# focegueda1998/CALM-ViT-DTE

Measured on AMD Instinct MI355X. Metric: training images/sec (224^2, bs=256/GPU), higher is better.
Workload: dtype f32; 1 GPU; CALM-ViT small224 cls, 224x224x3 synthetic, bs=256/GPU, fp32 matmuls, fwd+loss+bwd+clip+AdamW; batch resident in HBM when the timed region starts (the trainer's H2D copy of the batch is excluded); global_batch=256, parallelism=dp1, world=1, backend=none (single process), hipgraph=False

## Files before the change

calm-vit-dte_amd/Vi_Tools_CNN_less_V2.py:

```python
from functools import partial
from typing import Callable

import torch

from . import ops
from .backend import ACT_GELU, ACT_NONE, lean_forward
from .spectral_norm import SNConv2d, SNLinear, sn_scope


class ResidualStateManager():

    def __init__(self, smooth_factor: float = 2.0, momentum: float = 0.9, mode: str = "ema"):
        super().__init__()
        self.zq_sum = None
        self.zkv_sum = None
        self.tot_kl_loss = 0.0
        self.count = 0
        self.smooth_factor = smooth_factor
        self.mode = mode
        self.momentum = momentum

    @staticmethod
    def _kl(mean, std):
        return -0.5 * torch.mean(1 + 2 * torch.log(std) - mean.pow(2) - std.pow(2))
# ... 159 lines not shown
        self.rope_q = RoPE(seq_len_new, d_rope, learned=True)
        self.rope_k = RoPE(seq_len_new, d_rope, learned=True)
        self.linear_mask = torch.nn.Sequential(
            SNLinear(seq_len_new, seq_len_new * 2, bias=True),
            GELU(),
            SNLinear(seq_len_new * 2, seq_len_new, bias=True),
        )
        self.out_proj = SNLinear(dim2, dim2)
        self.out_proj.layer_scaled = True
        self.dropout = torch.nn.Dropout(dropout)
        self.ln_2 = LayerNorm(dim2)
        self.mlp = None
        if use_mlp:
            self.mlp = torch.nn.Sequential(
                SNLinear(dim2, mlp_dim),
                GELU(),
                torch.nn.Dropout(dropout, inplace=False),
                SNLinear(mlp_dim, dim2),
            )
            self.mlp[3].layer_scaled = True

    @staticmethod
    def _seq(lin, x):
        return ops.SeqLinearFn.apply(x, lin.weight_orig, lin.weight_u, lin.weight_v, lin.sigma())

    def forward(self, input_q, input_kv=None, state_manager=None, mask=False):
        if not mask:
            raise AttributeError("'NoneType' object has no attribute 'unsqueeze' (mask=False is not a usable "
                                 "path of the reference; every caller passes mask=True)")
        with sn_scope(self):
            return self._forward(input_q, input_kv, state_manager)

    def _project_qkv(self, qz, kz, vz, out16=False):
        pq, pk, pv = self.q_proj, self.k_proj, self.v_proj
        pack = lambda *ps: [t for p_ in ps for t in (p_.weight_orig, p_.weight_u, p_.weight_v, p_.sigma())]
        same_shape = pq.weight_orig.shape == pk.weight_orig.shape == pv.weight_orig.shape
        if any(p_.bias is not None for p_ in (pq, pk, pv)) or not same_shape or not ops.GROUP_PROJECTIONS:
            return pq(qz, out16=out16), pk(kz, out16=out16), pv(vz, out16=out16)
        if qz is kz and kz is vz:
            return ops.SNLinearGroupFn.apply(qz, out16, *pack(pq, pk, pv))
        if kz is vz:
            k, v = ops.SNLinearGroupFn.apply(kz, out16, *pack(pk, pv))
            return pq(qz, out16=out16), k, v
        return pq(qz, out16=out16), pk(kz, out16=out16), pv(vz, out16=out16)

    def _forward(self, input_q, input_kv, state_manager):
        H = self.heads
        xq, residual = self.ln_q.with_skip(input_q)
        xkv = xq if input_kv is None else self.ln_kv(input_kv, gemm_only=True)
        qz = qr = xq
        kz = vz = kr = xkv
        if self.reduce:
            if self.t_reduce:
                xq = self._seq(self.t_encoder_q, xq)
                xkv = self._seq(self.t_encoder_kv, xkv)
            mv_q = self.encoder_q(xq)
            mv_kv = self.encoder_kv(xkv)
            mvh = mv_q.shape[-1] // 2
            nq = ops.draw_noise(mv_q[..., :mvh]) if self.training else None
            nkv = ops.draw_noise(mv_kv[..., :mvh]) if self.training else None
            zq, std_q, kl_q = ops.LatentFn.apply(mv_q, nq)
            zkv, std_kv, kl_kv = ops.LatentFn.apply(mv_kv, nkv)
            if state_manager is not None:
                zq, zkv = state_manager.get_sums(zq, zkv, mv_q[..., :mvh], std_q, mv_kv[..., :mvh], std_kv,
                                                 kl_q=kl_q, kl_kv=kl_kv)
            qr = qz = zq
            kz = vz = zkv
            if self.t_reduce:
                qz = self._seq(self.t_qz_upsample, qz)
                kz = self._seq(self.t_kz_upsample, kz)
                vz = self._seq(self.t_vz_upsample, vz)
                qr = self._seq(self.t_qr_proj, qr)
                kr = self._seq(self.t_kr_proj, kr)
        a16 = qz.shape[1] == kz.shape[1] and ops.use_attention16(qz.shape[1], H, self.head_dim)
        qz, kz, v = self._project_qkv(qz, kz, vz, out16=a16)
        if self.reduce:
            qr = self.qr_proj(qr, out16=a16)
            kr = self.kr_proj(kr, out16=a16)
            q = ops.RopeFn.apply(qz, qr, self.rope_q.inv_freq, H, a16)
            k = ops.RopeFn.apply(kz, kr, self.rope_k.inv_freq, H, a16)
        else:
            q = ops.RopeFn.apply(None, qz, self.rope_q.inv_freq, H, a16)
            k = ops.RopeFn.apply(None, kz, self.rope_k.inv_freq, H, a16)
        m0, m2 = self.linear_mask[0], self.linear_mask[2]
        attention = ops.LatentMaskAttention16Fn if a16 else ops.LatentMaskAttentionFn
        if not a16 and ops.use_attention_lse(q.shape[1], k.shape[1], H, self.head_dim):
            attention = ops.LatentMaskAttentionLseFn
        if lean_forward():
            x = ops.latent_mask_attention_infer(q, k, v, m0.weight_orig, m0.bias, m2.weight_orig, m2.bias,
                                                m0.sigma(), m2.sigma(), H)
        else:
            x = attention.apply(
                q, k, v, m0.weight_orig, m0.bias, m2.weight_orig, m2.bias,
                m0.weight_u, m0.weight_v, m0.sigma(), m2.weight_u, m2.weight_v, m2.sigma(), H)
        if residual.shape != (x.shape[0], x.shape[1], self.out_proj.out_features):
            if self.input_t_proj is not None:
                residual = self._seq(self.input_t_proj, residual)
            if self.input_proj is not None:
                residual = self.input_proj(residual)
        p_att = self.dropout.p if self.training else 0.0
        if p_att > 0:
            x = self.out_proj(x, ls=self.ls_att)
            x = ops.DropoutAddFn.apply(x, residual, p_att, ops.draw_dropout_key(x.device))
        else:
            x = self.out_proj(x, ls=self.ls_att, residual=residual)
        if self.mlp is None:
            return self.ln_2(x)
        y, x = self.ln_2.with_skip(x)
        l0, l3 = self.mlp[0], self.mlp[3]
        mlp_args = (y, l0.weight_orig, None, l3.weight_orig, None, self.ls_mlp, x,
                    l0.weight_u, l0.weight_v, l0.sigma(), l3.weight_u, l3.weight_v, l3.sigma())
        p_mlp = self.mlp[2].p if self.training else 0.0
        if p_mlp > 0:
            return ops.MlpFn.apply(*mlp_args, p_mlp, ops.draw_dropout_key(y.device))
        return ops.MlpFn.apply(*mlp_args, 0.0, None, lean_forward())


class CnnResidual(torch.nn.Sequential):

    def __init__(self, hidden_channels=32):
        super().__init__(
            SNConv2d(3, hidden_channels, kernel_size=1, groups=1, bias=True),
            GELU(),
            SNConv2d(hidden_channels, hidden_channels, kernel_size=3, padding=1, bias=True, groups=hidden_channels),
            GELU(),
# ... 131 lines not shown
```

calm-vit-dte_amd/_lib.py:

```python
import ctypes as C
import os

HERE = os.path.dirname(os.path.abspath(__file__))
LIB_PATH = os.environ.get("CALM_VIT_LIB") or os.path.join(HERE, "libcalmvit_hip.so")

ACT_NONE, ACT_GELU, ACT_GELU_BWD = 0, 1, 2
F32 = 0
ST_F32, ST_BF16, ST_FP8_E4M3, ST_FP8_E5M2 = 0, 1, 2, 3
E_INVAL, E_LAYOUT, E_UNSUPP = -1, -2, -3
ABI_VERSION = 7

_p = C.c_void_p
_i32 = C.c_int32
_i64 = C.c_int64
_f32 = C.c_float


class GemmArgs(C.Structure):
    _fields_ = [
        ("A", _p), ("B", _p), ("C", _p),
        ("M", _i32), ("N", _i32), ("K", _i32),
        ("batch0", _i32), ("batch1", _i32),
        ("a_rs", _i64), ("a_cs", _i64), ("a_b0", _i64), ("a_b1", _i64),
        ("b_rs", _i64), ("b_cs", _i64), ("b_b0", _i64), ("b_b1", _i64),
# ... 140 lines not shown
    "calm_attention_bwd_lse": (_i32, [_p] * 7 + [_i64] + [_p] * 4 + [_i32] * 5 + [_p]),
    "calm_attention_infer": (_i32, [_p] * 11 + [_i32] * 5 + [_p]),
    "calm_attention16_supported": (_i32, [_i32, _i32, _i32]),
    "calm_attention16_fwd": (_i32, [_p] * 16 + [_i32] * 4 + [_p]),
    "calm_attention16_bwd": (_i32, [_p] * 13 + [_i32] * 4 + [_p]),
    "calm_attention16_infer": (_i32, [_p] * 11 + [_i32] * 4 + [_p]),
    "calm_latent_fwd": (_i32, [_p, _p, _p, _p, _p, _i64, _i32, _p, _p]),
    "calm_latent_bwd": (_i32, [_p, _p, _p, _p, _p, _p, _i64, _i32, _p]),
    "calm_sn_plan": (_i32, [C.POINTER(SnLayer), _i32, _p, C.POINTER(SnPlanInfo)]),
    "calm_sn_power_iter": (_i32, [_p, C.POINTER(SnPlanInfo), _i32, _f32, _p, _p]),
    "calm_sn_weight_bwd": (_i32, [_p, _p, _p, _p, _p, _p, _p, _p, _i32, _i32, _p, _p]),
    "calm_optim_chunk_elems": (_i32, []),
    "calm_optim_step": (_i32, [_p, _i32, _p, _i32, _p, C.POINTER(OptimHparams), _p, _p, _p, _p, _p]),
    "calm_grad_accum": (_i32, [_p, _i32, _p, _i32, _p, _p, _i32, _p]),
    "calm_ema_chunk_elems": (_i32, []),
    "calm_ema_update": (_i32, [_p, _i32, _p, _i32, _f32, _i32, _p, _p, _p, _p]),
    "calm_ema_swap": (_i32, [_p, _i32, _p, _i32, _p]),
    "calm_snapshot_chunk_bytes": (_i32, []),
    "calm_snapshot_pack": (_i32, [_p, _i32, _p, _i32, _p, _i64, _p]),
    "calm_snapshot_unpack": (_i32, [_p, _i32, _p, _i32, _p, _i64, _p]),
    "calm_collate_mix": (_i32, [_p, _p, _p, _i32, _i32, _i32, _i32, _f32, _p, _p, _p, _p]),
    "calm_collate_crop_mix": (_i32, [_p, _i32, _i32, _p, _p, _p, _i32, _i32, _i32, _i32, _i32, _f32, _p, _p, _p, _p]),
    "calm_augment_collate": (_i32, [_p, _i32, _i32, _p, _p, _p, _i32, _i32, _i32, _i32, _i32, _f32, _p, _p, _p, _p]),
    "calm_resize_coeffs": (_i32, [_i32, _i32, _p, _p, _i32]),
    "calm_resize_u8": (_i32, [_p, _i64, _p, _p, _i32, _i32, _i32, _p]),
    "calm_resized_crop": (_i32, [_p, _i64, _p, _p, _i32, _i32, _i32, _i32, _p, _p, _p]),
    "calm_resized_crop_check": (_i32, [C.POINTER(RCropSample), _i64, _i32, _i32]),
    "calm_image_to_rows": (_i32, [_p, _p, _i32, _i32, _p]),
    "calm_rows_to_image": (_i32, [_p, _p, _i32, _i32, _p]),
    "calm_grid_transpose": (_i32, [_p, _p, _i32, _i32, _p]),
    "calm_dwconv3x3_fwd": (_i32, [_p, _p, _p, _p, _p, _p, _i32, _i32, _i32, _i32, _p]),
    "calm_dwconv3x3_bwd": (_i32, [_p, _p, _p, _p, _p, _p, _p, _i32, _i32, _i32, _p]),
    "calm_cnn_residual_fwd": (_i32, [_p] * 11 + [_i32, _i32, _i32, _i32, _p]),
    "calm_cnn_residual_bwd": (_i32, [_p] * 18 + [_i32, _i32, _i32, _i32, _p, _p]),
    "calm_add": (_i32, [_p, _p, _p, _i64, _p]),
    "calm_gelu_fwd": (_i32, [_p, _p, _i64, _p]),
    "calm_gelu_bwd": (_i32, [_p, _p, _p, _i64, _p]),
    "calm_colsum": (_i32, [_p, _p, _i64, _i32, _i32, _p, _p]),
    "calm_row_scale": (_i32, [_p, _p, _p, _i32, _i32, _i32, _p]),
    "calm_mean_seq_fwd": (_i32, [_p, _p, _i32, _i32, _i32, _p]),
    "calm_mean_seq_bwd": (_i32, [_p, _p, _i32, _i32, _i32, _p]),
    "calm_soft_ce_fwd": (_i32, [_p, _i64, _p, _i64, _p, _p, _p, _i32, _i32, _p, _p]),
    "calm_soft_ce_bwd": (_i32, [_p, _i64, _p, _i64, _p, _p, _p, _i32, _i32, _p]),
    "calm_huber_tokens_fwd": (_i32, [_p, _p, _f32, _p, _i32, _i32, _p, _p]),
    "calm_huber_tokens_bwd": (_i32, [_p, _p, _f32, _p, _p, _i32, _i32, _p]),
    "calm_top1_count": (_i32, [_p, _i64, _p, _p, _i32, _i32, _p]),
    "calm_eval_metrics": (_i32, [_p, _i64, _i32, _p, C.POINTER(_i32), _i32, _p, _p, _p, _i32, _i32, _p, _p]),
    "calm_recon_huber_rows_fwd": (_i32, [_p, _p, _f32, _p, _i64, _p, _p]),
    "calm_recon_huber_rows_bwd": (_i32, [_p, _p, _f32, _p, _p, _i64, _p]),
    "calm_recon_metrics": (_i32, [_p, _i32, _p, _i32, C.POINTER(_f32), C.POINTER(_f32), _f32, _i32, _p, _i32, _i32, _p, _p]),
    "calm_distill_fwd": (_i32, [_p, _i64, _p, _i64, _i32, _p, _i64, _f32, _f32, _i32, _p, _p, _p, _p, _i32, _i32, _p, _p]),
    "calm_distill_bwd": (_i32, [_p, _i64, _p, _i64, _i32, _p, _i64, _f32, _f32, _i32, _p, _p, _p, _i32, _i32, _p]),
    "calm_dropout": (_i32, [_p, _p, _p, _i64, _i64, _f32, _p, _i32, _i32, _i32, _p]),
}

_lib = None


def load():
    global _lib
    if _lib is not None:
        return _lib
    if not os.path.exists(LIB_PATH):
        raise RuntimeError(
            f"{LIB_PATH} is missing: build it with `python -c 'import __graft_entry__ as g; g.build()'` "
            "(hipcc --offload-arch=gfx950).  The CALM-ViT path has no non-HIP fallback.")
    lib = C.CDLL(LIB_PATH)
    for name, (res, args) in SIGNATURES.items():
        fn = getattr(lib, name)
        fn.restype = res
        fn.argtypes = args
    if lib.calm_abi_version() != ABI_VERSION:
        raise RuntimeError("libcalmvit_hip.so ABI version mismatch")
    _lib = lib
    return lib


def check(rc, what):
    if rc != 0:
        kind = "invalid argument/unsupported shape" if rc < 0 else "hipError_t"
        raise RuntimeError(f"{what} failed: code {rc} ({kind})")
```

calm-vit-dte_amd/backend.py:

```python
import contextlib
import ctypes as C
import os

import numpy as np
import torch

from . import _lib
from ._lib import ACT_GELU, ACT_GELU_BWD, ACT_NONE

SN_EPS = 1e-12

GEMM_WORKSPACE = os.environ.get("CALM_GEMM_WORKSPACE", "1") != "0"
BF16_STORAGE = os.environ.get("CALM_BF16_STORAGE", "1") != "0"
PRECISIONS = {"fp32": 0, "bf16": 1, "bf16x3": 2, "fp8": 1}
FP8_DTYPES = (torch.float8_e4m3fn, torch.float8_e5m2)
_precision = "fp32"


def set_matmul_precision(name):
    global _precision
    if name not in PRECISIONS:
        raise ValueError(f"unknown matmul precision {name!r}; choose from {sorted(PRECISIONS)}")
    _precision = name

# ... 38 lines not shown
def lean_forward():
    return _lean_inference and not torch.is_grad_enabled()


_loss_kernels = os.environ.get("CALM_LOSS_KERNELS", "0") not in ("", "0")


def set_loss_kernels(on):
    global _loss_kernels
    _loss_kernels = bool(on)


def get_loss_kernels():
    return _loss_kernels


def loss_kernels_take(t):
    return _loss_kernels and t.dtype == torch.float32 and (t.is_cuda or not isinstance(get_backend(), HipBackend))


def eval_kernels_take(t):
    return (_loss_kernels and t.dtype in (torch.float32, torch.bfloat16)
            and (t.is_cuda or not isinstance(get_backend(), HipBackend)))


def recon_kernels_take(tokens, target):
    return eval_kernels_take(tokens) and target.dtype == torch.float32 and target.device == tokens.device


def effective_precision():
    if torch.is_autocast_enabled("cuda"):
        dt = torch.get_autocast_dtype("cuda")
        if dt != torch.bfloat16:
            raise NotImplementedError(f"autocast dtype {dt} is not supported on this path (the reference uses bfloat16)")
        return "bf16"
    return "bf16" if _precision == "fp8" else _precision


def fp8_linears():
    return _precision == "fp8" and BF16_STORAGE


def _ptr(t, allow_none=False, bf16_ok=False, fp8_ok=False):
    if t is None:
        if allow_none:
            return None
        raise ValueError("required tensor is None")
    if not t.is_cuda:
        raise RuntimeError("CALM-ViT ops run only on the MI355X HIP path: got a CPU tensor "
                           "(there is no CPU fallback; move the model and inputs to 'cuda')")
    if t.dtype != torch.float32 and not (bf16_ok and t.dtype == torch.bfloat16) and not (fp8_ok and t.dtype in FP8_DTYPES):
        raise TypeError(f"fp32 tensor expected, got {t.dtype}")
    return t.data_ptr()


def _ptr16(t):
    if t is None or not t.is_cuda or t.dtype != torch.bfloat16 or not t.is_contiguous():
        raise TypeError("contiguous bf16 CUDA tensor expected")
    return t.data_ptr()


_ST_OF = {torch.bfloat16: _lib.ST_BF16, torch.float8_e4m3fn: _lib.ST_FP8_E4M3, torch.float8_e5m2: _lib.ST_FP8_E5M2}


def _st(t):
    if t is None:
        return _lib.ST_F32
    return _ST_OF.get(t.dtype, _lib.ST_F32)


def bf16_pipeline():
    return BF16_STORAGE and effective_precision() == "bf16"


def act_dtype(last_dim):
    return torch.bfloat16 if bf16_pipeline() and last_dim % 8 == 0 else torch.float32


_raw_stream = getattr(torch._C, "_cuda_getCurrentRawStream", None)
_cur_device = getattr(torch._C, "_cuda_getDevice", None)


def _stream():
    if _raw_stream is not None:
        return _raw_stream(_cur_device())
    return torch.cuda.current_stream().cuda_stream


def chunk_table(lengths, chunk):
    chunk0, chunk_entry = [], []
    for i, n in enumerate(lengths):
        chunk0.append(len(chunk_entry))
        chunk_entry += [i] * ((n + chunk - 1) // chunk)
    return chunk0, chunk_entry


def _disjoint(spans):
    spans = sorted(spans)
    return not any(b[0] < a[1] for a, b in zip(spans, spans[1:]))


class ChunkPlan:

    def _tables(self, rec, lengths, chunk, dev):
        chunk0, chunk_entry = chunk_table(lengths, chunk)
        rec["chunk0"] = chunk0
# ... 845 lines not shown
        if partials is None:
            part = self._partials(_lib.RED_RECON, B, S, tokens.device)
        else:
            if partials.numel() < self.recon_scratch_floats(B, S):
                raise ValueError("recon_metrics: partials is smaller than calm_reduce_scratch_floats(CALM_RED_RECON, B, S)")
            part = _ptr(partials)
        m3, s3 = (_lib.C.c_float * 3)(*[float(v) for v in mean]), (_lib.C.c_float * 3)(*[float(v) for v in std])
        _lib.check(self.lib.calm_recon_metrics(_ptr(tokens, bf16_ok=True), _st(tokens), _ptr(target), int(layout), m3, s3,
                                               float(delta), int(bool(want_ssim)), sums.data_ptr(), B, S, part, _stream()),
                   "calm_recon_metrics")

    def recon_scratch_floats(self, B, S):
        need = self._scratch_need.get((_lib.RED_RECON, B, S))
        if need is None:
            need = self._scratch_need[(_lib.RED_RECON, B, S)] = int(self.lib.calm_reduce_scratch_floats(_lib.RED_RECON, B, S))
        return need

    def dropout(self, x, residual, y, n, p, key, e0=0):
        if key is None or not key.is_cuda or key.dtype != torch.int64 or key.numel() != 2 or not key.is_contiguous():
            raise TypeError("dropout expects its key as a contiguous int64 CUDA tensor of two elements (seed, offset)")
        _lib.check(self.lib.calm_dropout(_ptr(x, bf16_ok=True), _ptr(residual, True, bf16_ok=True), _ptr(y, bf16_ok=True),
                                         n, e0, float(p), key.data_ptr(), _st(x), _st(residual), _st(y), _stream()),
                   "calm_dropout")

    def add(self, a, b, out, n):
        _lib.check(self.lib.calm_add(_ptr(a), _ptr(b), _ptr(out), n, _stream()), "calm_add")

    def gelu_fwd(self, x, y, n):
        _lib.check(self.lib.calm_gelu_fwd(_ptr(x), _ptr(y), n, _stream()), "calm_gelu_fwd")

    def gelu_bwd(self, dy, z, dz, n):
        _lib.check(self.lib.calm_gelu_bwd(_ptr(dy), _ptr(z), _ptr(dz), n, _stream()), "calm_gelu_bwd")

    def colsum(self, x, out, rows, cols):
        _lib.check(self.lib.calm_colsum(_ptr(x, bf16_ok=True), _ptr(out), rows, cols, _st(x),
                                        self._partials(_lib.RED_COLSUM, rows, cols, x.device), _stream()), "calm_colsum")

    def colsum_part(self, x, rows, cols):
        part, shape = self._own_partials(_lib.RED_COLSUM, rows, cols, x.device), _lib.ReduceShape()
        _lib.check(self.lib.calm_part_colsum(_ptr(x, bf16_ok=True), rows, cols, _st(x), _ptr(part), C.byref(shape),
                                             _stream()), "calm_part_colsum")
        return part, shape

    def row_scale(self, x, s, out, rows, cols):
        _lib.check(self.lib.calm_row_scale(_ptr(x), _ptr(s), _ptr(out, bf16_ok=True), rows, cols, _st(out), _stream()),
                   "calm_row_scale")

    def mean_seq_fwd(self, x, y, B, S, D):
        _lib.check(self.lib.calm_mean_seq_fwd(_ptr(x), _ptr(y), B, S, D, _stream()), "calm_mean_seq_fwd")

    def mean_seq_bwd(self, dy, dx, B, S, D):
        _lib.check(self.lib.calm_mean_seq_bwd(_ptr(dy), _ptr(dx), B, S, D, _stream()), "calm_mean_seq_bwd")


_backend = None


def get_backend():
    global _backend
    if _backend is None:
        _backend = HipBackend()
    return _backend


@contextlib.contextmanager
def use_backend(b):
    global _backend
    old = _backend
    _backend = b
    try:
        yield b
    finally:
        _backend = old
```

calm-vit-dte_amd/build.py:

```python
import os
import shutil
import subprocess

HERE = os.path.dirname(os.path.abspath(__file__))
CSRC = os.path.join(HERE, "csrc")
LIB = os.path.join(HERE, "libcalmvit_hip.so")
SOURCES = ["gemm.hip", "gemm_f32.hip", "gemm_bf16.hip", "gemm_bf16p_kk.hip", "gemm_bf16p_km.hip", "gemm_bf16p_mm.hip", "gemm_f32p_kk.hip", "gemm_f32p_km.hip", "gemm_f32p_mm.hip", "gemm_fp8.hip", "norm_act.hip", "spectral.hip", "tokens_conv.hip", "cnn_fused.hip",
           "attention_fused.hip", "attention_bf16.hip", "optim.hip", "accum.hip", "ema.hip", "snapshot.hip", "loss.hip", "recon.hip", "dropout.hip", "augment.hip", "resize.hip", "resized_crop.hip"]
FLAGS = ["--offload-arch=gfx950", "-O3", "-fPIC", "-std=c++17", "-Wall", "-Wno-unused-function"]


def _hipcc():
    for cand in (os.environ.get("HIPCC"), shutil.which("hipcc"), "/opt/rocm/bin/hipcc"):
        if cand and os.path.exists(cand):
            return cand
    raise RuntimeError("hipcc not found: the CALM-ViT HIP library cannot be built")


def _stale(target, deps):
    if not os.path.exists(target):
        return True
    t = os.path.getmtime(target)
    return any(os.path.getmtime(d) > t for d in deps)


def build_library(force=False, verbose=False):
    hipcc = _hipcc()
    headers = [os.path.join(CSRC, h) for h in os.listdir(CSRC) if h.endswith(".h")]
    headers.append(os.path.join(HERE, "..", "include", "calm_vit.h"))
    objdir = os.path.join(HERE, "build")
    os.makedirs(objdir, exist_ok=True)
    objs, jobs = [], []
    for src in SOURCES:
        s = os.path.join(CSRC, src)
        o = os.path.join(objdir, src.replace(".hip", ".o"))
        if force or _stale(o, [s] + headers):
            cmd = [hipcc] + FLAGS + ["-c", s, "-o", o]
            if verbose:
                print(" ".join(cmd))
            jobs.append((src, subprocess.Popen(cmd)))
        objs.append(o)
    failed = [src for src, pr in jobs if pr.wait() != 0]
    if failed:
        raise RuntimeError(f"hipcc failed for {failed}")
    if force or _stale(LIB, objs):
        cmd = [hipcc, "--offload-arch=gfx950", "-shared", "-fPIC", "-o", LIB] + objs
        if verbose:
            print(" ".join(cmd))
        subprocess.run(cmd, check=True)
    return LIB


if __name__ == "__main__":
    print(build_library(verbose=True))
```

calm-vit-dte_amd/ops.py:

```python
import math
import os
import threading

import torch
from torch.autograd import Function
from torch.autograd.function import once_differentiable

from . import _lib
from .backend import (ACT_GELU, ACT_GELU_BWD, ACT_NONE, act_dtype, bf16_pipeline, effective_precision, fp8_linears,
                      get_attention_storage, get_backend)
from .spectral_norm import W16_ATTR, W16_GEN_ATTR

_amp_fwd = torch.amp.custom_fwd(device_type="cuda")
_amp_bwd = torch.amp.custom_bwd(device_type="cuda")

GROUP_PROJECTIONS = os.environ.get("CALM_GROUP_PROJECTIONS", "1") != "0"
FUSE_LN_SKIP = os.environ.get("CALM_FUSE_LN_SKIP", "1") != "0"

_noise_override = None


def set_noise_override(fn):
    global _noise_override
    _noise_override = fn
# ... 520 lines not shown
        ctx.wops = (wop1, wop2)
        ctx.wgen = _wgen(w1, w2)
        ctx.has_b1, ctx.has_b2, ctx.has_res = b1 is not None, b2 is not None, residual is not None
        ctx.biases = (_leaf(b1), _leaf(b2))
        ctx.defer = (_deferred(w1), _deferred(w2))
        ctx.xshape = x.shape
        ctx.save_for_backward(x2, hp, hg, w1, w2, ls, u1, v1, s1, u2, v2, s2, key if ctx.p > 0 else None)
        return out

    @staticmethod
    @once_differentiable
    @_amp_bwd
    def backward(ctx, dout):
        be = get_backend()
        x2, hp, hg, w1, w2, ls, u1, v1, s1, u2, v2, s2, key = ctx.saved_tensors
        _check_wgen(ctx.wgen, w1, w2)
        N, Hd = w2.shape
        K = w1.shape[1]
        do2 = _c(dout).reshape(-1, N)
        do2g = _gop(be, do2)
        G2 = _zeros_big(w2.shape, w2)
        _lin_wgrad(be, do2g, hg, G2)
        dW2, d_ls = _sn_wbwd(be, G2, w2, u2, v2, s2, ls, defer=ctx.defer[1])
        db2 = _colsum(be, do2, ctx.biases[1]) if ctx.has_b2 else None
        wop1, wop2 = ctx.wops
        if ls is not None:
            w2l = torch.empty_like(w2 if ctx.fp8 else wop2)
            be.row_scale(w2, ls, w2l, N, Hd)
        else:
            w2l = w2 if ctx.fp8 else wop2
        dhp = torch.empty_like(hp)
        if ctx.fp8:
            _lin_dgrad8(be, do2, w2l, s2, dhp, act=ACT_GELU_BWD, aux=hp)
        else:
            _lin_dgrad(be, do2g, w2l, s2, dhp, act=ACT_GELU_BWD, aux=hp)
        if ctx.p > 0:
            be.dropout(dhp, None, dhp, dhp.numel(), ctx.p, key)
        G1 = _zeros_big(w1.shape, w1)
        _lin_wgrad(be, dhp, x2, G1)
        dW1, _ = _sn_wbwd(be, G1, w1, u1, v1, s1, defer=ctx.defer[0])
        db1 = _colsum(be, dhp, ctx.biases[0]) if ctx.has_b1 else None
        dx = None
        if ctx.needs_input_grad[0]:
            dx = torch.empty_like(x2)
            if ctx.fp8:
                _lin_dgrad8(be, dhp, w1, s1, dx)
            else:
                _lin_dgrad(be, dhp, wop1, s1, dx)
            dx = dx.view(ctx.xshape)
        dres = dout if ctx.has_res else None
        return dx, dW1, db1, dW2, db2, d_ls, dres, None, None, None, None, None, None, None, None, None


class SeqLinearFn(Function):

    @staticmethod
    @_amp_fwd
    def forward(ctx, x, w, u, v, sigma):
        be = get_backend()
        x = _c(x)
        B, S, D = x.shape
        S2 = w.shape[0]
        wop = _wop(w)
        out = torch.empty(B, S2, D, dtype=torch.float32, device=x.device)
        be.gemm(wop, x, out, S2, D, S, (S, 1, 0, 0), (1, D, S * D, 0), (D, S2 * D, 0), batch=(B, 1), inv_scale=sigma)
        ctx.defer = _deferred(w)
        ctx.wop = wop
        ctx.wgen = _wgen(w)
        ctx.save_for_backward(x, w, u, v, sigma)
        return out

    @staticmethod
    @once_differentiable
    @_amp_bwd
    def backward(ctx, dy):
        be = get_backend()
        x, w, u, v, sigma = ctx.saved_tensors
        _check_wgen(ctx.wgen, w)
        B, S, D = x.shape
        S2 = w.shape[0]
        dy = _c(dy)
        dx = None
        if ctx.needs_input_grad[0]:
            dx = torch.empty_like(x)
            be.gemm(ctx.wop, dy, dx, S, D, S2, (1, S, 0, 0), (1, D, S2 * D, 0), (D, S * D, 0), batch=(B, 1),
                    inv_scale=sigma)
        G = _zeros_big(w.shape, w)
        be.gemm(dy, x, G, S2, S, D, (D, 1, S2 * D, 0), (D, 1, S * D, 0), (S, 0, 0), batch=(B, 1), reduce_batch=True,
                accumulate=True)
        dW, _ = _sn_wbwd(be, G, w, u, v, sigma, defer=ctx.defer)
        return dx, dW, None, None, None


class RopeFn(Function):

    @staticmethod
    @_amp_fwd
    def forward(ctx, content, xr, inv_freq, H, out16=False):
        be = get_backend()
        xr = _c(xr)
        B, S, W = xr.shape
        dr = W // H
        dc = 0
        if content is not None:
            content = _c(content)
            dc = content.shape[-1] // H
        table = torch.empty(2 * S * (dr // 2), dtype=torch.float32, device=xr.device)
        out = torch.empty(B, S, H * (dc + dr), dtype=torch.bfloat16 if out16 else torch.float32, device=xr.device)
        be.rope_fwd(content, xr, inv_freq, table, out, B, S, H, dc, dr)
        ctx.dims = (B, S, H, dc, dr)
        ctx.content_dtype = content.dtype if content is not None else None
        ctx.inv_freq = _leaf(inv_freq)
        ctx.save_for_backward(xr, table)
        return out

    @staticmethod
    @once_differentiable
    @_amp_bwd
    def backward(ctx, dout):
        be = get_backend()
        xr, table = ctx.saved_tensors
        B, S, H, dc, dr = ctx.dims
        dout = _c(dout)
        d_xr = torch.empty_like(xr)
        d_content = torch.empty(B, S, H * dc, dtype=ctx.content_dtype, device=xr.device) if dc > 0 else None
        d_if = _zeros((dr // 2,), table)
        if ctx.inv_freq is not None and _tail.takes(be, ctx.inv_freq):
            part, shape = be.rope_bwd_part(dout, xr, table, d_content, d_xr, B, S, H, dc, dr)
            _tail.add_reduce(part, shape, [d_if], (ctx.inv_freq,))
        else:
            be.rope_bwd(dout, xr, table, d_content, d_xr, d_if, B, S, H, dc, dr)
        return d_content, d_xr, d_if, None, None


def _attn_mask_bwd(be, defer, dM, q, k, dq, dk, R, hp, hg, w1, w2, u1, v1, s1, u2, v2, s2, w1o=None, w2o=None,
                   fold=False, biases=(None, None)):
    w1o, w2o = w1 if w1o is None else w1o, w2 if w2o is None else w2o
    B, Sq, D = q.shape
    Skv = k.shape[1]
    dev, dt = q.device, q.dtype
    G2 = _zeros_big(w2.shape, w2)
    _lin_wgrad(be, dM, hg, G2)
    dW2, _ = _sn_wbwd(be, G2, w2, u2, v2, s2, defer=defer[1])
    db2 = _colsum(be, dM, biases[1])
# ... 621 lines not shown
```

include/calm_vit.h:

```cpp
#ifndef CALM_VIT_H
#define CALM_VIT_H

#include <stddef.h>
#include <stdint.h>

#ifdef __cplusplus
extern "C" {
#endif

#define CALM_ABI_VERSION 7

#define CALM_E_INVAL   (-1)
#define CALM_E_LAYOUT  (-2)
#define CALM_E_UNSUPP  (-3)

enum { CALM_F32 = 0, CALM_BF16 = 1, CALM_BF16X3 = 2 };
enum { CALM_ST_F32 = 0, CALM_ST_BF16 = 1, CALM_ST_FP8_E4M3 = 2, CALM_ST_FP8_E5M2 = 3 };
enum { CALM_ACT_NONE = 0, CALM_ACT_GELU = 1, CALM_ACT_GELU_BWD = 2 };

int         calm_abi_version(void);
const char* calm_build_info(void);

typedef struct calm_gemm_args {
    const void* A; const void* B; void* C;
// ... 311 lines not shown
                          void* stream);

int calm_add(const float* a, const float* b, float* out, int64_t n, void* stream);
int calm_gelu_fwd(const float* x, float* y, int64_t n, void* stream);
int calm_gelu_bwd(const float* dy, const float* z, float* dz, int64_t n, void* stream);
int calm_colsum(const void* x, float* out, int64_t rows, int32_t cols, int32_t x_type ,
                float* partials , void* stream);
int calm_row_scale(const float* x, const float* s, void* out, int32_t rows, int32_t cols, int32_t out_type ,
                   void* stream);
int calm_mean_seq_fwd(const float* x, float* y, int32_t B, int32_t S, int32_t D, void* stream);
int calm_mean_seq_bwd(const float* dy, float* dx, int32_t B, int32_t S, int32_t D, void* stream);

int calm_dropout(const void* x, const void* residual , void* y, int64_t n, int64_t e0, float p,
                 const uint64_t* key , int32_t x_type, int32_t r_type, int32_t y_type,
                 void* stream);

int calm_soft_ce_fwd(const float* logits, int64_t ld, const float* targets, int64_t td,
                     float* row_stats ,
                     float* loss , float* metrics ,
                     int32_t B, int32_t C, float* partials, void* stream);
int calm_soft_ce_bwd(const float* logits, int64_t ld, const float* targets, int64_t td, const float* row_stats,
                     const float* dloss, float* dlogits , int32_t B, int32_t C, void* stream);
int calm_huber_tokens_fwd(const float* tokens, const float* x, float delta, float* loss, int32_t B, int32_t S,
                          float* partials, void* stream);
int calm_huber_tokens_bwd(const float* tokens, const float* x, float delta, const float* dloss, float* dtokens,
                          int32_t B, int32_t S, void* stream);
int calm_top1_count(const float* logits, int64_t ld, const int64_t* labels, float* metrics, int32_t B, int32_t C, void* stream);

int calm_eval_metrics(const void* logits, int64_t ld, int32_t logits_type, const int64_t* labels, const int32_t* ks,
                      int32_t nk, int64_t* counts, double* loss_sum, int64_t* confusion , int32_t B, int32_t C,
                      float* partials, void* stream);

enum { CALM_RECON_ROWS = 0, CALM_RECON_NCHW = 1 };
int calm_recon_huber_rows_fwd(const float* tokens, const float* target, float delta, float* loss ,
                              int64_t n, float* partials, void* stream);
int calm_recon_huber_rows_bwd(const float* tokens, const float* target, float delta, const float* dloss, float* dtokens,
                              int64_t n, void* stream);
int calm_recon_metrics(const void* tokens, int32_t tokens_type, const float* target, int32_t target_layout,
                       const float* mean , const float* std , float delta, int32_t want_ssim,
                       double* sums , int32_t B, int32_t S, float* partials, void* stream);

enum { CALM_DISTILL_SOFT = 0, CALM_DISTILL_HARD = 1 };
#define CALM_DISTILL_ROW_STATS 8
int calm_distill_fwd(const float* logits, int64_t ld, const void* teacher, int64_t tld, int32_t teacher_type,
                     const float* targets, int64_t td, float temperature, float alpha, int32_t mode,
                     float* row_stats , float* loss ,
                     float* metrics , float* dmetrics , int32_t B, int32_t C,
                     float* partials, void* stream);
int calm_distill_bwd(const float* logits, int64_t ld, const void* teacher, int64_t tld, int32_t teacher_type,
                     const float* targets, int64_t td, float temperature, float alpha, int32_t mode,
                     const float* row_stats, const float* dloss , float* dlogits ,
                     int32_t B, int32_t C, void* stream);

#ifdef __cplusplus
}
#endif
#endif
```

Measured before the change: 1977 images/sec.

## Add grouped sequence-mixing linear kernels and batch shared-input token projections

Adds a dedicated HIP kernel family for sequence-axis linear layers: forward and dgrad keep the small weight in LDS and use MFMA, and wgrad splits the batch reduction across workgroups with a partials buffer. Only the wgrad route is enabled by default for short sequences. The attention block now groups sequence projections that share an input (encoder q/kv, qz/qr upsample, kz/vz upsample) into one autograd function, so the grouped path runs several weights per launch. This aims to cut launch count and the poor utilisation of generic batched GEMMs on tiny S×S weights, at the cost of extra scratch memory and a separate reduction pass.

```diff
diff --git a/calm-vit-dte_amd/Vi_Tools_CNN_less_V2.py b/calm-vit-dte_amd/Vi_Tools_CNN_less_V2.py
--- a/calm-vit-dte_amd/Vi_Tools_CNN_less_V2.py
+++ b/calm-vit-dte_amd/Vi_Tools_CNN_less_V2.py
@@ -235,8 +235,11 @@
         kz = vz = kr = xkv
         if self.reduce:
             if self.t_reduce:
-                xq = self._seq(self.t_encoder_q, xq)
-                xkv = self._seq(self.t_encoder_kv, xkv)
+                if input_kv is None:
+                    xq, xkv = ops.seq_linear_group(xq, [self.t_encoder_q, self.t_encoder_kv])
+                else:
+                    xq = self._seq(self.t_encoder_q, xq)
+                    xkv = self._seq(self.t_encoder_kv, xkv)
             mv_q = self.encoder_q(xq)
             mv_kv = self.encoder_kv(xkv)
             mvh = mv_q.shape[-1] // 2
@@ -250,10 +253,8 @@
             qr = qz = zq
             kz = vz = zkv
             if self.t_reduce:
-                qz = self._seq(self.t_qz_upsample, qz)
-                kz = self._seq(self.t_kz_upsample, kz)
-                vz = self._seq(self.t_vz_upsample, vz)
-                qr = self._seq(self.t_qr_proj, qr)
+                qz, qr = ops.seq_linear_group(zq, [self.t_qz_upsample, self.t_qr_proj])
+                kz, vz = ops.seq_linear_group(zkv, [self.t_kz_upsample, self.t_vz_upsample])
                 kr = self._seq(self.t_kr_proj, kr)
         a16 = qz.shape[1] == kz.shape[1] and ops.use_attention16(qz.shape[1], H, self.head_dim)
         qz, kz, v = self._project_qkv(qz, kz, vz, out16=a16)
diff --git a/calm-vit-dte_amd/_lib.py b/calm-vit-dte_amd/_lib.py
--- a/calm-vit-dte_amd/_lib.py
+++ b/calm-vit-dte_amd/_lib.py
@@ -216,6 +216,11 @@
     "calm_distill_fwd": (_i32, [_p, _i64, _p, _i64, _i32, _p, _i64, _f32, _f32, _i32, _p, _p, _p, _p, _i32, _i32, _p, _p]),
     "calm_distill_bwd": (_i32, [_p, _i64, _p, _i64, _i32, _p, _i64, _f32, _f32, _i32, _p, _p, _p, _i32, _i32, _p]),
     "calm_dropout": (_i32, [_p, _p, _p, _i64, _i64, _f32, _p, _i32, _i32, _i32, _p]),
+    "calm_seq_linear_supported": (_i32, [_i32, _i32, _i32, _i32]),
+    "calm_seq_linear_scratch_floats": (_i64, [_i32, _i32, _i32, _i32, _i32]),
+    "calm_seq_linear_fwd": (_i32, [_p, _p, _p, _p, _i32, _i32, _i32, _i32, _i32, _p]),
+    "calm_seq_linear_dgrad": (_i32, [_p, _p, _p, _p, _i32, _i32, _i32, _i32, _i32, _p]),
+    "calm_seq_linear_wgrad": (_i32, [_p, _p, _p, _i32, _i32, _i32, _i32, _i32, _i32, _p, _i64, _p]),
 }
 
 _lib = None
diff --git a/calm-vit-dte_amd/backend.py b/calm-vit-dte_amd/backend.py
--- a/calm-vit-dte_amd/backend.py
+++ b/calm-vit-dte_amd/backend.py
@@ -114,6 +114,12 @@
     if t.dtype != torch.float32 and not (bf16_ok and t.dtype == torch.bfloat16) and not (fp8_ok and t.dtype in FP8_DTYPES):
         raise TypeError(f"fp32 tensor expected, got {t.dtype}")
     return t.data_ptr()
+
+
+def _contig(t):
+    if not t.is_contiguous():
+        raise ValueError("contiguous tensor expected")
+    return t
 
 
 def _ptr16(t):
@@ -1065,6 +1071,41 @@
     def mean_seq_bwd(self, dy, dx, B, S, D):
         _lib.check(self.lib.calm_mean_seq_bwd(_ptr(dy), _ptr(dx), B, S, D, _stream()), "calm_mean_seq_bwd")
 
+    def seq_linear_supported(self, S2, S, D, G):
+        key = ("seq", S2, S, D, G)
+        ok = self._scratch_need.get(key)
+        if ok is None:
+            ok = self._scratch_need[key] = bool(self.lib.calm_seq_linear_supported(S2, S, D, G))
+        return ok
+
+    @staticmethod
+    def _ptrs(ts):
+        return (C.c_void_p * len(ts))(*[_ptr(_contig(t)) for t in ts])
+
+    def seq_linear_fwd(self, x, ws, sigmas, ys, B, S2, S, D):
+        _lib.check(self.lib.calm_seq_linear_fwd(_ptr(_contig(x)), self._ptrs(ws), self._ptrs(sigmas), self._ptrs(ys), len(ws),
+                                                B, S2, S, D, _stream()), "calm_seq_linear_fwd")
+
+    def seq_linear_dgrad(self, dys, ws, sigmas, dx, B, S2, S, D):
+        _lib.check(self.lib.calm_seq_linear_dgrad(self._ptrs(dys), self._ptrs(ws), self._ptrs(sigmas), _ptr(_contig(dx)),
+                                                  len(ws), B, S2, S, D, _stream()), "calm_seq_linear_dgrad")
+
+    def seq_linear_wgrad(self, dys, x, grs, B, S2, S, D, accumulate=True):
+        G = len(dys)
+        key = ("seqw", B, S2, S, D, G)
+        need = self._scratch_need.get(key)
+        if need is None:
+            need = self._scratch_need[key] = int(self.lib.calm_seq_linear_scratch_floats(B, S2, S, D, G))
+        skey = (x.device.index, _stream())
+        buf = self._scratch_bufs.get(skey)
+        if buf is None or buf.numel() < need:
+            if buf is not None:
+                self._scratch_retired.append(buf)
+            buf = self._scratch_bufs[skey] = torch.empty(max(need, 1 << 20), dtype=torch.float32, device=x.device)
+        _lib.check(self.lib.calm_seq_linear_wgrad(self._ptrs(dys), _ptr(_contig(x)), self._ptrs(grs), G, B, S2, S, D,
+                                                  int(accumulate), buf.data_ptr(), buf.numel(), _stream()),
+                   "calm_seq_linear_wgrad")
+
 
 _backend = None
 
diff --git a/calm-vit-dte_amd/build.py b/calm-vit-dte_amd/build.py
--- a/calm-vit-dte_amd/build.py
+++ b/calm-vit-dte_amd/build.py
@@ -6,7 +6,7 @@
 CSRC = os.path.join(HERE, "csrc")
 LIB = os.path.join(HERE, "libcalmvit_hip.so")
 SOURCES = ["gemm.hip", "gemm_f32.hip", "gemm_bf16.hip", "gemm_bf16p_kk.hip", "gemm_bf16p_km.hip", "gemm_bf16p_mm.hip", "gemm_f32p_kk.hip", "gemm_f32p_km.hip", "gemm_f32p_mm.hip", "gemm_fp8.hip", "norm_act.hip", "spectral.hip", "tokens_conv.hip", "cnn_fused.hip",
-           "attention_fused.hip", "attention_bf16.hip", "optim.hip", "accum.hip", "ema.hip", "snapshot.hip", "loss.hip", "recon.hip", "dropout.hip", "augment.hip", "resize.hip", "resized_crop.hip"]
+           "attention_fused.hip", "attention_bf16.hip", "optim.hip", "accum.hip", "ema.hip", "snapshot.hip", "loss.hip", "recon.hip", "dropout.hip", "augment.hip", "resize.hip", "resized_crop.hip", "seq_linear.hip"]
 FLAGS = ["--offload-arch=gfx950", "-O3", "-fPIC", "-std=c++17", "-Wall", "-Wno-unused-function"]
 
 
diff --git a/calm-vit-dte_amd/csrc/seq_linear.hip b/calm-vit-dte_amd/csrc/seq_linear.hip
--- /dev/null
+++ b/calm-vit-dte_amd/csrc/seq_linear.hip
@@ -0,0 +1,370 @@
+#include "common.h"
+
+namespace {
+
+#define MFMA16(a, b, c) __builtin_amdgcn_mfma_f32_16x16x4f32((a), (b), (c), 0, 0, 0)
+
+constexpr int SL_WAVES = 8, SL_THREADS = 64 * SL_WAVES;
+constexpr int SL_MAX_G = 3;
+constexpr int SL_CUS = 256;
+constexpr long SL_LDS_MAX = 160 * 1024;
+constexpr int SL_MAX_DIM = 4096;
+constexpr int SL_WG_TILES = 4;
+
+inline int ceil_to(int v, int m) { return (v + m - 1) / m * m; }
+inline int sl_ld(int rows16) { return rows16 + ((rows16 % 32 == 16) ? 0 : 16); }
+inline long sl_lds_bytes(int M, int K, int G) { return 4L * G * ceil_to(K, 4) * sl_ld(ceil_to(M, 16)); }
+
+struct SeqP {
+    const float* in[SL_MAX_G];
+    float* out[SL_MAX_G];
+    const float* w[SL_MAX_G];
+    const float* sigma[SL_MAX_G];
+    int G, M, K, D;
+    int S;
+    int kp, ldm, mtiles, slabs, passes;
+    long items;
+};
+
+template <int MT, int KU>
+__device__ __forceinline__ void sl_kloop(const float* __restrict__ xb, bool dok, const SeqP& p, const float* wl, int mt0,
+                                         int q, int r, f32x4 (&acc)[MT][4]) {
+    const f32x4 zero = {0.f, 0.f, 0.f, 0.f};
+    f32x4 xc[KU], xn[KU];
+    auto load4 = [&](f32x4 (&x)[KU], int k0) {
+#pragma unroll
+        for (int u = 0; u < KU; ++u) {
+            const int k = k0 + 4 * u + q;
+            x[u] = (dok && k < p.K) ? *reinterpret_cast<const f32x4*>(xb + (long)k * p.D) : zero;
+        }
+    };
+    load4(xc, 0);
+    for (int k0 = 0; k0 < p.kp; k0 += 4 * KU) {
+        if (k0 + 4 * KU < p.kp) load4(xn, k0 + 4 * KU);
+#pragma unroll
+        for (int u = 0; u < KU; ++u) {
+            if (k0 + 4 * u < p.kp) {
+                const float* wk = wl + (k0 + 4 * u + q) * p.ldm + 16 * mt0 + r;
+#pragma unroll
+                for (int i = 0; i < MT; ++i) {
+                    if (mt0 + i < p.mtiles) {
+                        const float a = wk[16 * i];
+#pragma unroll
+                        for (int e = 0; e < 4; ++e) acc[i][e] = MFMA16(a, xc[u][e], acc[i][e]);
+                    }
+                }
+            }
+        }
+#pragma unroll
+        for (int u = 0; u < KU; ++u) xc[u] = xn[u];
+    }
+}
+
+template <int MT, bool TRANS, bool SUM>
+__global__ __launch_bounds__(SL_THREADS) void seq_linear_kernel(const SeqP p) {
+    extern __shared__ __attribute__((aligned(16))) float sl_smem[];
+    const int tid = threadIdx.x, lane = tid & 63;
+    const int wave = __builtin_amdgcn_readfirstlane(tid >> 6);
+    const int r = lane & 15, q = lane >> 4;
+    const int mp = 16 * p.mtiles, img = p.kp * p.ldm;
+    for (int g = 0; g < p.G; ++g) {
+        float* dst = sl_smem + g * img;
+        const float* w = p.w[g];
+        constexpr int SB = 8;
+        const int total = p.kp * mp;
+        for (int base = tid; base < total; base += SB * SL_THREADS) {
+            float v[SB];
+            int off[SB];
+#pragma unroll
+            for (int u = 0; u < SB; ++u) {
+                const int idx = base + u * SL_THREADS;
+                const int hi = idx / (TRANS ? mp : p.kp), lo = idx - hi * (TRANS ? mp : p.kp);
+                const int k = TRANS ? hi : lo, m = TRANS ? lo : hi;
+                off[u] = idx < total ? k * p.ldm + m : -1;
+                v[u] = (idx < total && k < p.K && m < p.M) ? w[(long)hi * p.S + lo] : 0.f;
+            }
+#pragma unroll
+            for (int u = 0; u < SB; ++u)
+                if (off[u] >= 0) dst[off[u]] = v[u];
+        }
+    }
+    __syncthreads();
+    float inv[SL_MAX_G];
+#pragma unroll
+    for (int g = 0; g < SL_MAX_G; ++g) inv[g] = g < p.G ? 1.0f / p.sigma[g][0] : 0.f;
+
+    const f32x4 zero = {0.f, 0.f, 0.f, 0.f};
+    for (long it = (long)blockIdx.x * SL_WAVES + wave; it < p.items; it += (long)gridDim.x * SL_WAVES) {
+        const long sb = it / p.passes, b = sb / p.slabs;
+        const int mt0 = (int)(it - sb * p.passes) * MT;
+        const int d = (int)(sb - b * p.slabs) * 64 + 4 * r;
+        const bool dok = d < p.D;
+        const long in_off = b * p.K * p.D + d, out_off = b * p.M * p.D + d;
+        {
+            f32x4 tot[SUM ? MT : 1][4];
+#pragma unroll
+            for (int g = 0; g < SL_MAX_G; ++g) {
+                if (g < p.G) {
+                    f32x4 acc[MT][4];
+#pragma unroll
+                    for (int i = 0; i < MT; ++i)
+#pragma unroll
+                        for (int e = 0; e < 4; ++e) acc[i][e] = zero;
+                    sl_kloop<MT, (MT > 4 || SUM) ? 4 : 8>(p.in[TRANS ? g : 0] + in_off, dok, p, sl_smem + g * img, mt0, q, r, acc);
+                    if constexpr (SUM) {
+#pragma unroll
+                        for (int i = 0; i < MT; ++i)
+#pragma unroll
+                            for (int e = 0; e < 4; ++e) tot[i][e] = g == 0 ? acc[i][e] * inv[0] : tot[i][e] + acc[i][e] * inv[g];
+                    }
+                    if (!SUM || g == p.G - 1) {
+                        float* ob = p.out[TRANS ? 0 : g] + out_off;
+#pragma unroll
+                        for (int i = 0; i < MT; ++i) {
+#pragma unroll
+                            for (int j = 0; j < 4; ++j) {
+                                const int m = 16 * (mt0 + i) + 4 * q + j;
+                                if (dok && mt0 + i < p.mtiles && m < p.M) {
+                                    f32x4 v;
+#pragma unroll
+                                    for (int e = 0; e < 4; ++e) {
+                                        if constexpr (SUM) v[e] = tot[i][e][j];
+                                        else v[e] = acc[i][e][j] * inv[g];
+                                    }
+                                    *reinterpret_cast<f32x4*>(ob + (long)m * p.D) = v;
+                                }
+                            }
+                        }
+                    }
+                }
+            }
+        }
+    }
+}
+
+struct SeqWP {
+    const float* dy[SL_MAX_G];
+    const float* x;
+    float* part;
+    int G, S2, S, D;
+    int mt, nt, mch, nch;
+    int dchunks;
+    long items, per;
+};
+
+__global__ __launch_bounds__(SL_THREADS) void seq_linear_wgrad_kernel(const SeqWP p) {
+    constexpr int T = SL_WG_TILES;
+    __shared__ f32x4 red[SL_WAVES / 2][T * T][64];
+    const int tid = threadIdx.x, lane = tid & 63;
+    const int wave = __builtin_amdgcn_readfirstlane(tid >> 6);
+    const int r = lane & 15, q = lane >> 4;
+    const int blocks = p.mch * p.nch, pairs = p.G * blocks;
+    const int pair = blockIdx.x % pairs, slice = blockIdx.x / pairs;
+    const int g = pair / blocks, mc = (pair - g * blocks) / p.nch, nc = pair - g * blocks - mc * p.nch;
+    const int mt0 = mc * T, nt0 = nc * T;
+    const float* __restrict__ dy = p.dy[g];
+    const float* __restrict__ x = p.x;
+    const f32x4 zero = {0.f, 0.f, 0.f, 0.f};
+    f32x4 acc[T][T];
+#pragma unroll
+    for (int i = 0; i < T; ++i)
+#pragma unroll
+        for (int j = 0; j < T; ++j) acc[i][j] = zero;
+
+    const long first = slice * p.per, last = first + p.per < p.items ? first + p.per : p.items;
+    f32x4 a[T], bx[T], an[T], bn[T];
+    auto load = [&](f32x4 (&av)[T], f32x4 (&bv)[T], long it) {
+        const long b = it / p.dchunks;
+        const int d = (int)(it - b * p.dchunks) * 16 + 4 * q;
+        const bool ok = it < last && d < p.D;
+#pragma unroll
+        for (int i = 0; i < T; ++i) {
+            const int m = 16 * (mt0 + i) + r;
+            av[i] = (ok && m < p.S2) ? *reinterpret_cast<const f32x4*>(dy + (b * p.S2 + m) * p.D + d) : zero;
+        }
+#pragma unroll
+        for (int j = 0; j < T; ++j) {
+            const int n = 16 * (nt0 + j) + r;
+            bv[j] = (ok && n < p.S) ? *reinterpret_cast<const f32x4*>(x + (b * p.S + n) * p.D + d) : zero;
+        }
+    };
+    load(a, bx, first + wave);
+    for (long it = first + wave; it < last; it += SL_WAVES) {
+        load(an, bn, it + SL_WAVES);
+#pragma unroll
+        for (int e = 0; e < 4; ++e)
+#pragma unroll
+            for (int i = 0; i < T; ++i)
+                if (mt0 + i < p.mt) {
+#pragma unroll
+                    for (int j = 0; j < T; ++j)
+                        if (nt0 + j < p.nt) acc[i][j] = MFMA16(a[i][e], bx[j][e], acc[i][j]);
+                }
+#pragma unroll
+        for (int i = 0; i < T; ++i) { a[i] = an[i]; bx[i] = bn[i]; }
+    }
+#pragma unroll
+    for (int half = SL_WAVES / 2; half >= 1; half >>= 1) {
+        __syncthreads();
+        if (wave >= half && wave < 2 * half) {
+#pragma unroll
+            for (int i = 0; i < T; ++i)
+#pragma unroll
+                for (int j = 0; j < T; ++j) red[wave - half][i * T + j][lane] = acc[i][j];
+        }
+        __syncthreads();
+        if (wave < half) {
+#pragma unroll
+            for (int i = 0; i < T; ++i)
+#pragma unroll
+                for (int j = 0; j < T; ++j) acc[i][j] += red[wave][i * T + j][lane];
+        }
+    }
+    if (wave == 0) {
+        float* dst = p.part + ((long)slice * p.G + g) * p.S2 * p.S;
+#pragma unroll
+        for (int i = 0; i < T; ++i)
+#pragma unroll
+            for (int j = 0; j < T; ++j) {
+                const int n = 16 * (nt0 + j) + r;
+#pragma unroll
+                for (int e = 0; e < 4; ++e) {
+                    const int m = 16 * (mt0 + i) + 4 * q + e;
+                    if (m < p.S2 && n < p.S) dst[(long)m * p.S + n] = acc[i][j][e];
+                }
+            }
+    }
+}
+
+struct WgradPlan {
+    int mt, nt, mch, nch, pairs, nslice, dchunks;
+    long items, per;
+};
+WgradPlan plan_wgrad(long B, int S2, int S, int D, int G) {
+    WgradPlan w;
+    w.mt = (S2 + 15) / 16; w.nt = (S + 15) / 16;
+    w.mch = (w.mt + SL_WG_TILES - 1) / SL_WG_TILES; w.nch = (w.nt + SL_WG_TILES - 1) / SL_WG_TILES;
+    w.pairs = G * w.mch * w.nch;
+    w.dchunks = (D + 15) / 16;
+    w.items = B * w.dchunks;
+    long want = SL_CUS / w.pairs;
+    const long most = (w.items + SL_WAVES - 1) / SL_WAVES;
+    if (want > most) want = most;
+    if (want < 1) want = 1;
+    w.per = (w.items + want - 1) / want;
+    w.nslice = (int)((w.items + w.per - 1) / w.per);
+    return w;
+}
+
+bool shape_ok(int S2, int S, int D, int G) {
+    return S2 > 0 && S > 0 && D > 0 && G >= 1 && G <= SL_MAX_G && S2 <= SL_MAX_DIM && S <= SL_MAX_DIM && D % 4 == 0 &&
+           sl_lds_bytes(S2, S, G) <= SL_LDS_MAX && sl_lds_bytes(S, S2, G) <= SL_LDS_MAX;
+}
+
+template <bool TRANS>
+int launch_seq(SeqP& p, long B, void* stream) {
+    p.kp = ceil_to(p.K, 4);
+    p.mtiles = (p.M + 15) / 16;
+    p.ldm = sl_ld(16 * p.mtiles);
+    p.slabs = (p.D + 63) / 64;
+    const int lds = (int)sl_lds_bytes(p.M, p.K, p.G);
+    const bool sum = TRANS && p.G > 1;
+    return with_int<3, 5, 4>(sum || p.mtiles == 3 ? 3 : p.mtiles == 5 ? 5 : 4, [&](auto mt) {
+        constexpr int MT = decltype(mt)::value;
+        p.passes = (p.mtiles + MT - 1) / MT;
+        p.items = B * p.slabs * p.passes;
+        long grid = (p.items + SL_WAVES - 1) / SL_WAVES;
+        if (grid > SL_CUS) grid = SL_CUS;
+        void (*kernel)(const SeqP) = seq_linear_kernel<MT, TRANS, false>;
+        if constexpr (TRANS && MT == 3) {
+            if (sum) kernel = seq_linear_kernel<3, true, true>;
+        }
+        hipError_t e = hipFuncSetAttribute(reinterpret_cast<const void*>(kernel), hipFuncAttributeMaxDynamicSharedMemorySize, lds);
+        if (e != hipSuccess) return (int)e;
+        return calm_launch(kernel, dim3((unsigned)grid), dim3(SL_THREADS), (size_t)lds, stream, p);
+    });
+}
+
+int check_shape(int G, int B, int S2, int S, int D) {
+    if (G <= 0 || B <= 0 || S2 <= 0 || S <= 0 || D <= 0) return CALM_E_INVAL;
+    if (!shape_ok(S2, S, D, G)) return CALM_E_UNSUPP;
+    return 0;
+}
+
+}
+
+extern "C" {
+
+int calm_seq_linear_supported(int32_t S2, int32_t S, int32_t D, int32_t G) { return shape_ok(S2, S, D, G) ? 1 : 0; }
+
+int64_t calm_seq_linear_scratch_floats(int32_t B, int32_t S2, int32_t S, int32_t D, int32_t G) {
+    if (B <= 0 || !shape_ok(S2, S, D, G)) return 0;
+    return (int64_t)plan_wgrad(B, S2, S, D, G).nslice * G * S2 * S;
+}
+
+int calm_seq_linear_fwd(const float* x, const float* const* w, const float* const* sigma, float* const* y, int32_t G,
+                        int32_t B, int32_t S2, int32_t S, int32_t D, void* stream) {
+    if (!x || !w || !sigma || !y) return CALM_E_INVAL;
+    if (int rc = check_shape(G, B, S2, S, D)) return rc;
+    SeqP p{};
+    for (int g = 0; g < G; ++g) {
+        if (!w[g] || !sigma[g] || !y[g]) return CALM_E_INVAL;
+        if (!aligned16(y[g])) return CALM_E_LAYOUT;
+        p.w[g] = w[g]; p.sigma[g] = sigma[g]; p.out[g] = y[g];
+    }
+    if (!aligned16(x)) return CALM_E_LAYOUT;
+    p.in[0] = x;
+    p.G = G; p.M = S2; p.K = S; p.D = D; p.S = S;
+    return launch_seq<false>(p, B, stream);
+}
+
+int calm_seq_linear_dgrad(const float* const* dy, const float* const* w, const float* const* sigma, float* dx, int32_t G,
+                          int32_t B, int32_t S2, int32_t S, int32_t D, void* stream) {
+    if (!dy || !w || !sigma || !dx) return CALM_E_INVAL;
+    if (int rc = check_shape(G, B, S2, S, D)) return rc;
+    SeqP p{};
+    for (int g = 0; g < G; ++g) {
+        if (!dy[g] || !w[g] || !sigma[g]) return CALM_E_INVAL;
+        if (!aligned16(dy[g])) return CALM_E_LAYOUT;
+        p.in[g] = dy[g]; p.w[g] = w[g]; p.sigma[g] = sigma[g];
+    }
+    if (!aligned16(dx)) return CALM_E_LAYOUT;
+    p.out[0] = dx;
+    p.G = G; p.M = S; p.K = S2; p.D = D; p.S = S;
+    return launch_seq<true>(p, B, stream);
+}
+
+int calm_seq_linear_wgrad(const float* const* dy, const float* x, float* const* gr, int32_t G, int32_t B, int32_t S2,
+                          int32_t S, int32_t D, int32_t accumulate, float* partials, int64_t partials_floats, void* stream) {
+    if (!dy || !x || !gr || !partials) return CALM_E_INVAL;
+    if (int rc = check_shape(G, B, S2, S, D)) return rc;
+    const WgradPlan w = plan_wgrad(B, S2, S, D, G);
+    const long n = (long)G * S2 * S;
+    if (partials_floats < w.nslice * n) return CALM_E_INVAL;
+    SeqWP p{};
+    for (int g = 0; g < G; ++g) {
+        if (!dy[g] || !gr[g]) return CALM_E_INVAL;
+        if (!aligned16(dy[g])) return CALM_E_LAYOUT;
+        p.dy[g] = dy[g];
+    }
+    if (!aligned16(x) || !aligned16(partials)) return CALM_E_LAYOUT;
+    p.x = x; p.part = partials;
+    p.G = G; p.S2 = S2; p.S = S; p.D = D;
+    p.mt = w.mt; p.nt = w.nt; p.mch = w.mch; p.nch = w.nch; p.dchunks = w.dchunks; p.items = w.items; p.per = w.per;
+    CalmReduceDst dst{};
+    for (int g = 0; g < G; ++g) {
+        dst.out[g] = gr[g];
+        dst.begin[g] = g * S2 * S;
+        if (!accumulate) {
+            hipError_t e = hipMemsetAsync(gr[g], 0, sizeof(float) * (size_t)S2 * S, as_stream(stream));
+            if (e != hipSuccess) return (int)e;
+        }
+    }
+    dst.begin[G] = (int)n;
+    dst.nseg = G;
+    if (int rc = calm_launch(seq_linear_wgrad_kernel, dim3((unsigned)(w.pairs * w.nslice)), dim3(SL_THREADS), 0, stream, p))
+        return rc;
+    return calm_reduce_partials(partials, w.nslice, (int)n, (int)n, dst, stream);
+}
+
+}
diff --git a/calm-vit-dte_amd/ops.py b/calm-vit-dte_amd/ops.py
--- a/calm-vit-dte_amd/ops.py
+++ b/calm-vit-dte_amd/ops.py
@@ -596,6 +596,31 @@
         return dx, dW1, db1, dW2, db2, d_ls, dres, None, None, None, None, None, None, None, None, None
 
 
+SEQ_LINEAR = os.environ.get("CALM_SEQ_LINEAR", "1") != "0"
+SEQ_LINEAR_SHORT = 80
+SEQ_LINEAR_OPS = frozenset(["wgrad"])
+
+
+def seq_linear_route(be, op, S2, S, D, G, *tensors):
+    return (SEQ_LINEAR and op in SEQ_LINEAR_OPS and hasattr(be, "seq_linear_" + op) and effective_precision() == "fp32"
+            and all(t.dtype == torch.float32 for t in tensors) and min(S2, S) <= SEQ_LINEAR_SHORT
+            and be.seq_linear_supported(S2, S, D, G))
+
+
+def _seq_fwd(be, x, wop, sigma, out, B, S2, S, D):
+    be.gemm(wop, x, out, S2, D, S, (S, 1, 0, 0), (1, D, S * D, 0), (D, S2 * D, 0), batch=(B, 1), inv_scale=sigma)
+
+
+def _seq_dgrad(be, dy, wop, sigma, dx, B, S2, S, D, accumulate=False):
+    be.gemm(wop, dy, dx, S, D, S2, (1, S, 0, 0), (1, D, S2 * D, 0), (D, S * D, 0), batch=(B, 1), inv_scale=sigma,
+            accumulate=accumulate)
+
+
+def _seq_wgrad(be, dy, x, G, B, S2, S, D):
+    be.gemm(dy, x, G, S2, S, D, (D, 1, S2 * D, 0), (D, 1, S * D, 0), (S, 0, 0), batch=(B, 1), reduce_batch=True,
+            accumulate=True)
+
+
 class SeqLinearFn(Function):
 
     @staticmethod
@@ -607,7 +632,10 @@
         S2 = w.shape[0]
         wop = _wop(w)
         out = torch.empty(B, S2, D, dtype=torch.float32, device=x.device)
-        be.gemm(wop, x, out, S2, D, S, (S, 1, 0, 0), (1, D, S * D, 0), (D, S2 * D, 0), batch=(B, 1), inv_scale=sigma)
+        if seq_linear_route(be, "fwd", S2, S, D, 1, x, w, wop, sigma):
+            be.seq_linear_fwd(x, [w], [sigma], [out], B, S2, S, D)
+        else:
+            _seq_fwd(be, x, wop, sigma, out, B, S2, S, D)
         ctx.defer = _deferred(w)
         ctx.wop = wop
         ctx.wgen = _wgen(w)
@@ -627,13 +655,94 @@
         dx = None
         if ctx.needs_input_grad[0]:
             dx = torch.empty_like(x)
-            be.gemm(ctx.wop, dy, dx, S, D, S2, (1, S, 0, 0), (1, D, S2 * D, 0), (D, S * D, 0), batch=(B, 1),
-                    inv_scale=sigma)
+            if seq_linear_route(be, "dgrad", S2, S, D, 1, x, dy, w, ctx.wop, sigma):
+                be.seq_linear_dgrad([dy], [w], [sigma], dx, B, S2, S, D)
+            else:
+                _seq_dgrad(be, dy, ctx.wop, sigma, dx, B, S2, S, D)
         G = _zeros_big(w.shape, w)
-        be.gemm(dy, x, G, S2, S, D, (D, 1, S2 * D, 0), (D, 1, S * D, 0), (S, 0, 0), batch=(B, 1), reduce_batch=True,
-                accumulate=True)
+        if seq_linear_route(be, "wgrad", S2, S, D, 1, x, dy):
+            be.seq_linear_wgrad([dy], x, [G], B, S2, S, D)
+        else:
+            _seq_wgrad(be, dy, x, G, B, S2, S, D)
         dW, _ = _sn_wbwd(be, G, w, u, v, sigma, defer=ctx.defer)
         return dx, dW, None, None, None
+
+
+class SeqLinearGroupFn(Function):
+
+    @staticmethod
+    @_amp_fwd
+    def forward(ctx, x, *wuvs):
+        be = get_backend()
+        n = len(wuvs) // 4
+        ws, sigmas = list(wuvs[0::4]), list(wuvs[3::4])
+        x = _c(x)
+        B, S, D = x.shape
+        S2 = ws[0].shape[0]
+        assert all(w.shape == (S2, S) for w in ws)
+        if effective_precision() != "fp32" or any(t.dtype != torch.float32 for t in (x, *ws, *sigmas)):
+            raise RuntimeError("SeqLinearGroupFn: fp32 steps on fp32 tensors only "
+                               "(ops.seq_linear_group chooses between the group and one SeqLinearFn per weight)")
+        outs = [torch.empty(B, S2, D, dtype=torch.float32, device=x.device) for _ in range(n)]
+        if seq_linear_route(be, "fwd", S2, S, D, n, x):
+            be.seq_linear_fwd(x, ws, sigmas, outs, B, S2, S, D)
+        else:
+            for g in range(n):
+                _seq_fwd(be, x, ws[g], sigmas[g], outs[g], B, S2, S, D)
+        ctx.n = n
+        ctx.wgen = _wgen(*ws)
+        ctx.defer = [_deferred(w) for w in ws]
+        ctx.set_materialize_grads(False)
+        ctx.save_for_backward(x, *wuvs)
+        return tuple(outs)
+
+    @staticmethod
+    @once_differentiable
+    @_amp_bwd
+    def backward(ctx, *dys):
+        be = get_backend()
+        x, *wuvs = ctx.saved_tensors
+        n = ctx.n
+        ws, us, vs, sigmas = list(wuvs[0::4]), list(wuvs[1::4]), list(wuvs[2::4]), list(wuvs[3::4])
+        _check_wgen(ctx.wgen, *ws)
+        B, S, D = x.shape
+        S2 = ws[0].shape[0]
+        live = [g for g in range(n) if dys[g] is not None]
+        dy = {g: _c(dys[g]) for g in live}
+        sub = lambda ts: [ts[g] for g in live]
+        grads = [None] * (4 * n)
+        dx = None
+        if ctx.needs_input_grad[0]:
+            if not live:
+                dx = torch.zeros_like(x)
+            else:
+                dx = torch.empty_like(x)
+                if seq_linear_route(be, "dgrad", S2, S, D, len(live), x, *sub(dy)):
+                    be.seq_linear_dgrad(sub(dy), sub(ws), sub(sigmas), dx, B, S2, S, D)
+                else:
+                    for i, g in enumerate(live):
+                        _seq_dgrad(be, dy[g], ws[g], sigmas[g], dx, B, S2, S, D, accumulate=i > 0)
+        if live:
+            Gs = {g: _zeros_big(ws[g].shape, ws[g]) for g in live}
+            if seq_linear_route(be, "wgrad", S2, S, D, len(live), x, *sub(dy)):
+                be.seq_linear_wgrad(sub(dy), x, sub(Gs), B, S2, S, D)
+            else:
+                for g in live:
+                    _seq_wgrad(be, dy[g], x, Gs[g], B, S2, S, D)
+            for g in live:
+                grads[4 * g] = _sn_wbwd(be, Gs[g], ws[g], us[g], vs[g], sigmas[g], defer=ctx.defer[g])[0]
+        return (dx, *grads)
+
+
+def seq_linear_group(x, lins):
+    pack = [t for lin in lins for t in (lin.weight_orig, lin.weight_u, lin.weight_v, lin.sigma())]
+    ws = pack[0::4]
+    S2, S = ws[0].shape
+    if (SEQ_LINEAR and len(lins) > 1 and hasattr(get_backend(), "seq_linear_fwd") and x.dim() == 3 and x.shape[1] == S
+            and all(w.shape == (S2, S) for w in ws) and effective_precision() == "fp32"
+            and all(t.dtype == torch.float32 for t in (x, *ws, *pack[3::4]))):
+        return list(SeqLinearGroupFn.apply(x, *pack))
+    return [SeqLinearFn.apply(x, *pack[4 * i:4 * i + 4]) for i in range(len(lins))]
 
 
 class RopeFn(Function):
diff --git a/include/calm_vit.h b/include/calm_vit.h
--- a/include/calm_vit.h
+++ b/include/calm_vit.h
@@ -387,6 +387,15 @@
                      const float* row_stats, const float* dloss , float* dlogits ,
                      int32_t B, int32_t C, void* stream);
 
+int calm_seq_linear_supported(int32_t S2, int32_t S, int32_t D, int32_t G);
+int64_t calm_seq_linear_scratch_floats(int32_t B, int32_t S2, int32_t S, int32_t D, int32_t G);
+int calm_seq_linear_fwd(const float* x, const float* const* w, const float* const* sigma, float* const* y, int32_t G,
+                        int32_t B, int32_t S2, int32_t S, int32_t D, void* stream);
+int calm_seq_linear_dgrad(const float* const* dy, const float* const* w, const float* const* sigma, float* dx, int32_t G,
+                          int32_t B, int32_t S2, int32_t S, int32_t D, void* stream);
+int calm_seq_linear_wgrad(const float* const* dy, const float* x, float* const* gr, int32_t G, int32_t B, int32_t S2,
+                          int32_t S, int32_t D, int32_t accumulate, float* partials, int64_t partials_floats, void* stream);
+
 #ifdef __cplusplus
 }
 #endif
```

Measured after the change: 1986 images/sec, median of 6. No clear change (+0.4%).
